# MILAB-IIT-CV/ATDN_vSLAM

Measured on AMD Instinct MI355X. Metric: frame-pairs/sec, KITTI 1241x376 odometry inference at 1/2/4/8 MI355X, higher is better.
Workload: dtype f32 via 3xf16 split MFMA (fp32 accumulate); 1 GPU; KITTI seq-03-shaped 376x1241 uint8 frames (resident in HBM) resized to 376x1232, GMA flow 12 GRU iters + CLVO head -> 6-DoF trajectory (BASELINE configs[1]); streams_per_gpu=2, gru_iters=12, parallelism=pairs sharded x1, one all-gather of 512-d features, replicated LSTM scan

## Files before the change

atdn_vslam_amd/csrc/capi.hip:

```cpp
#include "../../include/atdn_hip.h"

#include <cmath>
#include <cstring>

#include "clvo.h"
#include "gma.h"
#include "vae.h"
#include "clvo_train.h"
#include "frontend.h"
#include "conv_sf.h"
#include "epilogues_sf.h"

namespace atdn {
extern template TileChoice conv_dispatch<MODE_TAP, EpiBias<ACT_NONE>>(const ConvShape&, EpiBias<ACT_NONE>, hipStream_t);
extern template TileChoice conv_dispatch<MODE_TAP, EpiBias<ACT_RELU>>(const ConvShape&, EpiBias<ACT_RELU>, hipStream_t);
extern template TileChoice conv_dispatch<MODE_ROW, EpiBias<ACT_NONE>>(const ConvShape&, EpiBias<ACT_NONE>, hipStream_t);
extern template TileChoice conv_dispatch<MODE_ROW, EpiBias<ACT_RELU>>(const ConvShape&, EpiBias<ACT_RELU>, hipStream_t);
extern template TileChoice conv_dispatch<MODE_TAP, EpiScale>(const ConvShape&, EpiScale, hipStream_t);

extern template TileChoice conv_sf_dispatch<EpiBias<ACT_NONE>>(const ConvShape&, float, EpiBias<ACT_NONE>, hipStream_t);
extern template TileChoice conv_sf_dispatch<SfBias<ACT_NONE>>(const ConvShape&, float, SfBias<ACT_NONE>, hipStream_t);

static thread_local std::string g_last_error;
void set_last_error(const std::string& msg) { g_last_error = msg; }
// ... 518 lines not shown
  ATDN_API_BEGIN
  ATDN_CHECK(src && dst && planes >= 1 && Hin >= 1 && Win >= 1 && Hout >= 1 && Wout >= 1, "bad argument");
  ATDN_CHECK(antialias == 0 || antialias == 1, "antialias must be ATDN_RESIZE_BILINEAR or ATDN_RESIZE_ANTIALIAS");
  launch_resize<unsigned char>(src, planes, Hin, Win, Hout, Wout, antialias, dst, (hipStream_t)stream);
  ATDN_API_END
}
int atdn_pad_frames(const float* src, int planes, int H, int W, int left, int right, int top, int bottom, float* dst,
                    void* stream) {
  ATDN_API_BEGIN
  ATDN_CHECK(src && dst && planes >= 1 && H >= 1 && W >= 1 && left >= 0 && right >= 0 && top >= 0 && bottom >= 0, "bad argument");
  launch_pad_replicate(src, planes, H, W, left, right, top, bottom, dst, (hipStream_t)stream);
  ATDN_API_END
}
int atdn_ingest_create(atdn_ingest** out, int Hin, int Win, int Hout, int Wout, int max_frames, int antialias) {
  ATDN_API_BEGIN
  ATDN_CHECK(out, "null out pointer");
  ATDN_CHECK(antialias == 0 || antialias == 1, "antialias must be ATDN_RESIZE_BILINEAR or ATDN_RESIZE_ANTIALIAS");
  *out = new atdn_ingest(Hin, Win, Hout, Wout, max_frames, antialias);
  ATDN_API_END
}
int atdn_ingest_frames_u8(atdn_ingest* h, const uint8_t* host_frames, int n_frames, float* dst, void* stream) {
  ATDN_API_BEGIN
  ATDN_CHECK(h, "null handle");
  h->in.ingest(host_frames, n_frames, dst, (hipStream_t)stream);
  ATDN_API_END
}
void atdn_ingest_destroy(atdn_ingest* h) { delete h; }

int atdn_conv2d_nhwc_sf_epi(const float* src, int nimg, int H, int W, int Cin, const float* weight_host,
                            const float* bias_host, int Cout, int KH, int KW, int stride, int padH, int padW, int sf_store,
                            float* dst, void* stream) {
  ATDN_API_BEGIN
  ATDN_CHECK(src && weight_host && dst && nimg >= 1 && Cin % 32 == 0, "bad argument (Cin must be a multiple of 32)");
  ATDN_CHECK(!sf_store || Cout % 32 == 0, "the split-f16 store needs Cout % 32 == 0");
  StateDict sd;
  const int64_t ws[4] = {Cout, Cin, KH, KW};
  sd.put("c.weight", weight_host, ws, 4);
  std::vector<float> zb(Cout, 0.f);
  const int64_t bs[1] = {Cout};
  sd.put("c.bias", bias_host ? bias_host : zb.data(), bs, 1);
  WeightArena A;
  PackedConv L = pack_conv_sf(A, sd, {"c"});
  A.upload();
  resolve(A, L);
  hipStream_t st = (hipStream_t)stream;
  float* tmp = nullptr;
  const long rows = (long)nimg * H * W;
  ATDN_HIP(hipMalloc(&tmp, (size_t)rows * Cin * sizeof(float)));
  try {
    launch_to_sf(src, tmp, rows, Cin, st);
    ConvShape s;
    s.src0 = tmp; s.ld0 = Cin; s.sb0 = (long)H * W * Cin; s.C0 = L.C; s.H = H; s.W = W;
    s.KH = KH; s.KW = KW; s.stride = stride; s.padH = padH; s.padW = padW;
    s.w = L.w; s.ldw = L.ldw; s.N = Cout; s.nimg = nimg;
    const int Ho = conv_out(H, KH, stride, padH), Wo = conv_out(W, KW, stride, padW);
    s.wfrag16 = L.wf16;
    if (sf_store) {
      float* osf = nullptr;
      const long orows = (long)nimg * Ho * Wo;
      ATDN_HIP(hipMalloc(&osf, (size_t)orows * Cout * sizeof(float)));
      try {
        conv_sf_dispatch(s, L.wscale, SfBias<ACT_NONE>{L.b, osf, (long)Ho * Wo * Cout, Cout}, st);
        launch_from_sf(osf, dst, orows, Cout, st);
        ATDN_HIP(hipStreamSynchronize(st));
      } catch (...) {
        (void)hipFree(osf);
        throw;
      }
      (void)hipFree(osf);
    } else {
      conv_sf_dispatch(s, L.wscale, EpiBias<ACT_NONE>{L.b, dst, (long)Ho * Wo * Cout, Cout, 1.f}, st);
      ATDN_HIP(hipStreamSynchronize(st));
    }
  } catch (...) {
    (void)hipFree(tmp);
    A.release();
    throw;
  }
  (void)hipFree(tmp);
  A.release();
  ATDN_API_END
}

int atdn_conv2d_nhwc_sf(const float* src, int nimg, int H, int W, int Cin, const float* weight_host,
                        const float* bias_host, int Cout, int KH, int KW, int stride, int padH, int padW, float* dst,
                        void* stream) {
  return atdn_conv2d_nhwc_sf_epi(src, nimg, H, W, Cin, weight_host, bias_host, Cout, KH, KW, stride, padH, padW, 0, dst, stream);
}

// ... 2 lines not shown
```

atdn_vslam_amd/csrc/conv_mfma.h:

```cpp
#pragma once
#include "common.h"

namespace atdn {

typedef float f32x16 __attribute__((ext_vector_type(16)));

enum { MODE_TAP = 0, MODE_ROW = 1 };

struct ConvGeom {
  const float* src0;
  const float* src1;
  long sb0, sb1;
  int ld0, ld1;
  int C0, C1;
  int H, W, Ho, Wo;
  int KH, KW, stride, padH, padW;
  int cpk;
  int nchunks;
  int log2C;
  const float* w;
  long wb;
  int ldw;
  int N;
  int tiles_per_img, nimg, ntile_n;
// ... 182 lines not shown
          for (int e = 0; e < 16; ++e) {
            const int m = mbase + (e & 3) + 8 * (e >> 2) + 4 * h;
            if (m < HoWo) ep.apply(img, m, n, acc[i][j][e], aux[e]);
          }
        } else if constexpr (epi_bias_arg<Epi>::value) {
#pragma unroll
          for (int e = 0; e < 16; ++e) {
            const int m = mbase + (e & 3) + 8 * (e >> 2) + 4 * h;
            if (m < HoWo) ep.store_c(img, m, n, acc[i][j][e], colj[j]);
          }
        } else {
#pragma unroll
          for (int e = 0; e < 16; ++e) {
            const int m = mbase + (e & 3) + 8 * (e >> 2) + 4 * h;
            if (m < HoWo) ep(img, m, n, acc[i][j][e]);
          }
        }
      }
    }
  }
}

struct ConvShape {
  const float* src0 = nullptr; const float* src1 = nullptr;
  long sb0 = 0, sb1 = 0;
  int ld0 = 0, ld1 = 0, C0 = 0, C1 = 0;
  int H = 1, W = 1;
  int KH = 1, KW = 1, stride = 1, padH = 0, padW = 0;
  const float* w = nullptr; long wb = 0; int ldw = 0;
  const float* wfrag16 = nullptr;
  int N = 0;
  int nimg = 1;
  const float* in_mean = nullptr; const float* in_rstd = nullptr;
};

inline int conv_out(int in, int k, int stride, int pad) { return (in + 2 * pad - k) / stride + 1; }

template <int MODE>
inline ConvGeom make_geom(const ConvShape& s, int BM, int BN) {
  ConvGeom g{};
  g.src0 = s.src0; g.src1 = s.src1; g.sb0 = s.sb0; g.sb1 = s.sb1; g.ld0 = s.ld0; g.ld1 = s.ld1;
  g.C0 = s.C0; g.C1 = s.C1; g.H = s.H; g.W = s.W;
  g.KH = s.KH; g.KW = s.KW; g.stride = s.stride; g.padH = s.padH; g.padW = s.padW;
  g.Ho = conv_out(s.H, s.KH, s.stride, s.padH);
  g.Wo = conv_out(s.W, s.KW, s.stride, s.padW);
  if (MODE == MODE_TAP) {
    ATDN_CHECK(s.C0 % 32 == 0 && s.C1 % 32 == 0 && s.C0 > 0, "TAP mode needs channel counts that are multiples of 32");
    ATDN_CHECK(s.ld0 % 4 == 0 && (s.C1 == 0 || (s.src1 && s.ld1 % 4 == 0)), "TAP mode needs 16-byte aligned pixels");
    g.cpk = s.KW * ((s.C0 + s.C1) / 32);
    g.log2C = 0;
  } else {
    ATDN_CHECK(s.C1 == 0 && s.src1 == nullptr, "ROW mode takes one source");
    ATDN_CHECK(s.C0 >= 4 && (s.C0 & (s.C0 - 1)) == 0 && s.ld0 == s.C0, "ROW mode needs dense power-of-two channels");
    g.cpk = cdiv(s.KW * s.C0, 32);
    int l = 0; while ((1 << l) < s.C0) ++l;
    g.log2C = l;
  }
  g.nchunks = s.KH * g.cpk;
  g.w = s.w; g.wb = s.wb; g.ldw = s.ldw; g.N = s.N;
  ATDN_CHECK(s.ldw % 4 == 0 && s.ldw >= g.nchunks * 32, "weight rows must hold the padded K and be 16-byte aligned");
  ATDN_CHECK(((uintptr_t)s.src0 % 16) == 0 && ((uintptr_t)s.w % 16) == 0 && s.sb0 % 4 == 0 && s.wb % 4 == 0,
             "operands must be 16-byte aligned");
  ATDN_CHECK(g.Ho > 0 && g.Wo > 0 && s.N > 0 && s.nimg > 0, "empty convolution");
  g.nimg = s.nimg;
  g.tiles_per_img = cdiv(g.Ho * g.Wo, BM);
  g.ntile_n = cdiv(s.N, BN);
// ... 18 lines not shown
```

atdn_vslam_amd/csrc/conv_sf6.h:

```cpp
#pragma once
#include <cstdlib>
#include <type_traits>
#include "conv_sf.h"

namespace atdn {

struct Conv2Geom {
  const float* src0; const float* src1;
  long sb0, sb1;
  int ld0, ld1, C0, C1;
  int H, W, Ho, Wo;
  int KH, KW, padH, padW;
  int PH, PW;
  int tiles_x, tiles_y;
  int nimg, ntile_n;
  const float* w; int ldw; int N;
  float wscale;
  const float* in_mean; const float* in_rstd;
};

inline bool conv_halo_eligible(const ConvShape& s) {
  if (s.stride != 1 || s.wb != 0) return false;
  return (s.KH == 3 && s.KW == 3) || (s.KH == 1 && s.KW == 5) || (s.KH == 5 && s.KW == 1);
}

template <class E, class = void> struct epi_gen6 : std::integral_constant<int, 0> {};
template <class E> struct epi_gen6<E, std::void_t<decltype(E::kGen6)>> : std::integral_constant<int, E::kGen6> {};
template <class E, class = void> struct EpiAux4 { struct type {}; };
template <class E> struct EpiAux4<E, std::void_t<typename E::Aux4>> { using type = typename E::Aux4; };
template <class E, class = void> struct epi_flowhead : std::false_type {};
template <class E> struct epi_flowhead<E, std::void_t<decltype(E::kFlowHead)>> : std::bool_constant<E::kFlowHead> {};
template <class E, class = void> struct epi_ring3 : std::false_type {};
template <class E> struct epi_ring3<E, std::void_t<decltype(E::kRing3)>> : std::bool_constant<E::kRing3> {};
template <class E, class = void> struct epi_rawacc : std::false_type {};
template <class E> struct epi_rawacc<E, std::void_t<decltype(E::kRawAcc)>> : std::bool_constant<E::kRawAcc> {};
template <class E, class = void> struct epi_vec4 : std::false_type {};
template <class E> struct epi_vec4<E, std::void_t<decltype(E::kVec4)>> : std::bool_constant<E::kVec4> {};

typedef float f32x4v __attribute__((ext_vector_type(4)));
struct SfAcc { f32x4v b[2][2]; };

#ifdef ATDN_CONV_STAMP
#define ATDN_CONV_STAMP_SLOTS 4096
extern __device__ unsigned long long atdn_conv_stamps_dev[4][ATDN_CONV_STAMP_SLOTS][12];
template <class E> struct conv_stamp_kind : std::integral_constant<int, -1> {};
#endif

template <int TH, int TW, int BN, int WM, int WN, int KH, int KW, class Epi, bool FAST = false, bool NORM = false, int ABL = 0>
__device__ __forceinline__ void conv_sf6_body(const Conv2Geom& g, const Epi& ep, const int bidx) {
  static_assert(ABL == 0 || !NORM, "ablation builds exist for the plain patch loader");
  static_assert(TW == 16, "the 16x16x32 loop is built for 16-pixel tile rows");
  constexpr int NIMG = 2;
  constexpr int NW = WM * WN, NT = NW * 64;
  constexpr int TM = TH * TW / 32 / WM, TN = BN / 32 / WN;
  static_assert(TM * WM * 32 == TH * TW && TN * WN * 32 == BN, "wave grid must tile the block");
  static_assert(32 % TW == 0 || TW % 32 == 0, "a 32-pixel MFMA row tile must cover whole tile rows");
  constexpr int NTAP = KH * KW;
  constexpr int RSTEP = NT / 8;
  constexpr int PROWS = (TH + KH - 1) * (TW + KW - 1);
  constexpr int PW = TW + KW - 1;
  constexpr int NP = (PROWS + RSTEP - 1) / RSTEP;
  constexpr int ROWB = 160;
  constexpr int RS = PW * ROWB;
  constexpr bool SWAP = epi_vec4<Epi>::value;
  constexpr int PSZ = (TH + KH - 1) * RS;
  __shared__ __attribute__((aligned(256))) char Pbytes[NIMG * PSZ];

  const int tid = threadIdx.x;
  const int tiles_img = g.tiles_x * g.tiles_y;
  const int nblk = g.nimg * tiles_img * g.ntile_n;
  const int id = xcd_remap(bidx, nblk);
  const int tile_n = id % g.ntile_n;
  const int tmg = id / g.ntile_n;
  const int img = tmg / tiles_img;
  const int tloc = tmg - img * tiles_img;
  const int ty0 = (tloc / g.tiles_x) * TH, tx0 = (tloc % g.tiles_x) * TW;
  const int n0 = tile_n * BN;
  const int lane = tid & 63, wave = tid >> 6;
#ifdef ATDN_CONV_STAMP
  constexpr int kStamp = conv_stamp_kind<Epi>::value;
  unsigned long long st_r0 = 0, st_t0 = 0, st_t1 = 0, st_t2 = 0, st_bar = 0;
  unsigned long long st_e_slab = 0, st_e_wait = 0, st_e_apply = 0;
  if constexpr (kStamp >= 0) { st_r0 = __builtin_amdgcn_s_memrealtime(); st_t0 = __builtin_amdgcn_s_memtime(); }
#endif

  const int jrow = (tid >> 3) & 7;
  const int s = tid & 7, r0 = !NORM ? tid >> 3 : ((tid >> 6) << 3) + 2 * (jrow & 1) + ((jrow >> 1) & 1) + 4 * (jrow >> 2);
  static_assert((TH + KH - 1) * RS / 16 <= 4096, "LDS offset field");
  unsigned pmeta[NP];
#pragma unroll
  for (int k = 0; k < NP; ++k) {
    const int prow = r0 + RSTEP * k;
    unsigned off = 0;
    const int py = prow / PW, px = prow - py * PW;
    if (prow < PROWS) {
      const int iy = ty0 - g.padH + py, ix = tx0 - g.padW + px;
      if ((unsigned)iy < (unsigned)g.H && (unsigned)ix < (unsigned)g.W) off = (unsigned)(iy * g.W + ix) + 1u;
    }
    pmeta[k] = (off << 12) | (unsigned)((py * RS + px * ROWB + 16 * s) >> 4);
    if (prow >= PROWS) pmeta[k] = pmeta[0];
  }
  const float* s0 = g.src0 + (long)img * g.sb0;
  const float* s1 = g.src1 ? g.src1 + (long)img * g.sb1 : nullptr;
  const int nck = (g.C0 + g.C1) >> 5;

  float4 pr[NP];
  auto fetch_patch = [&](int c) {
    const int cc = c << 5;
    const float* sp; int ld, co;
    if (cc < g.C0) { sp = s0; ld = g.ld0; co = cc; } else { sp = s1; ld = g.ld1; co = cc - g.C0; }
#pragma unroll
    for (int k = 0; k < NP; ++k)
      pr[k] = *reinterpret_cast<const float4*>(sp + (long)((pmeta[k] >> 12) ? (pmeta[k] >> 12) - 1 : 0) * ld + co + 4 * s);
  };
  auto store_patch = [&](int buf) {
#pragma unroll
    for (int k = 0; k < NP; ++k)
      *reinterpret_cast<float4*>(Pbytes + buf * PSZ + ((pmeta[k] & 0xFFFu) << 4)) = keep_if((pmeta[k] >> 12) != 0, pr[k]);
  };
  float4 nmu = make_float4(0.f, 0.f, 0.f, 0.f), nrs = make_float4(1.f, 1.f, 1.f, 1.f);
  auto fetch_norm = [&](int c) {
    nmu = *reinterpret_cast<const float4*>(g.in_mean + (long)img * g.C0 + (c << 5) + 4 * s);
    nrs = *reinterpret_cast<const float4*>(g.in_rstd + (long)img * g.C0 + (c << 5) + 4 * s);
  };
  bool norm_sat = false;
  auto store_row_norm = [&](int buf, int k, float4 mu, float4 rs) {
    const float hi = (pmeta[k] >> 12) != 0 ? 65504.f : 0.f;
    float4 v = pr[k];
    v.x = (v.x - mu.x) * rs.x; v.y = (v.y - mu.y) * rs.y; v.z = (v.z - mu.z) * rs.z; v.w = (v.w - mu.w) * rs.w;
    const float m = fmaxf(fmaxf(v.x, v.y), fmaxf(v.z, v.w));
    norm_sat |= !(m <= 65504.f);
    v.x = __builtin_amdgcn_fmed3f(v.x, 0.f, hi); v.y = __builtin_amdgcn_fmed3f(v.y, 0.f, hi);
    v.z = __builtin_amdgcn_fmed3f(v.z, 0.f, hi); v.w = __builtin_amdgcn_fmed3f(v.w, 0.f, hi);
    const unsigned h0 = sf_cvt_pk_(v.x, v.y), h1 = sf_cvt_pk_(v.z, v.w);
    const unsigned l0 = sf_residual_pk_(h0, v.x, v.y), l1 = sf_residual_pk_(h1, v.z, v.w);
    char* px = Pbytes + buf * PSZ + (((pmeta[k] & 0xFFFu) - (unsigned)s) << 4);
    *reinterpret_cast<uint2*>(px + 8 * s) = make_uint2(h0, h1);
    *reinterpret_cast<uint2*>(px + 64 + 8 * s) = make_uint2(l0, l1);
  };

  const int wm = wave / WN, wn = wave % WN;
  SfAcc acc[TM][TN];
#pragma unroll
  for (int i = 0; i < TM; ++i)
#pragma unroll
    for (int j = 0; j < TN; ++j) {
#pragma unroll
      for (int e = 0; e < 16; ++e) acc[i][j].b[e >> 3][(e >> 2) & 1][e & 3] = 0.f;
    }
  {
    const int n16 = lane & 15, g16 = lane >> 4;
    int a_off[TM];
#pragma unroll
    for (int i = 0; i < TM; ++i) a_off[i] = ((wm * TM + i) * 2) * RS + n16 * ROWB + 16 * g16;
    const char* Pb = Pbytes;
    const int nblk16 = (g.N + 15) >> 4;
    const float* wrow[TN][2];
#pragma unroll
    for (int j = 0; j < TN; ++j)
#pragma unroll
      for (int cb = 0; cb < 2; ++cb)
        wrow[j][cb] = g.w + (long)min(((n0 >> 4) + (wn * TN + j) * 2 + cb), nblk16 - 1) * (NTAP * nck) * 512 + lane * 4;
    constexpr int RT = (NTAP % 3 == 0 || epi_ring3<Epi>::value) ? 3 : 2;
    constexpr int CU = (NTAP % RT == 0) ? 1 : RT;
    constexpr int NS = CU * NTAP;
    static_assert(NS % RT == 0, "ring size must divide the K steps of an unrolled iteration");
    struct WFrag { f16x8 hi[TN][2], lo[TN][2]; };
    WFrag wr[RT];
    auto load_w = [&](WFrag& f, int c0, int st, int cb) __attribute__((always_inline)) {
      const int cc = min(c0 + st / NTAP, nck - 1);
      const int q = (st % NTAP) * nck + cc;
#pragma unroll
      for (int j = 0; j < TN; ++j) {
        f.hi[j][cb] = *reinterpret_cast<const f16x8*>(wrow[j][cb] + (long)q * 512);
        if constexpr (!FAST) f.lo[j][cb] = *reinterpret_cast<const f16x8*>(wrow[j][cb] + (long)q * 512 + 256);
      }
    };
    fetch_patch(0);
    if constexpr (NORM) fetch_norm(0);
#pragma unroll
    for (int st = 0; st < RT - 1; ++st) { load_w(wr[st], 0, st, 0); load_w(wr[st], 0, st, 1); }
    if constexpr ((ABL & 1) != 0) { load_w(wr[RT - 1], 0, RT - 1, 0); load_w(wr[RT - 1], 0, RT - 1, 1); }
    if constexpr (NORM) {
#pragma unroll
      for (int k = 0; k < NP; ++k) store_row_norm(0, k, nmu, nrs);
    } else {
      store_patch(0);
    }
    __syncthreads();
#ifdef ATDN_CONV_STAMP
    if constexpr (kStamp >= 0) st_t1 = __builtin_amdgcn_s_memtime();
#endif
    f16x8 ah[2][TM], al[2][TM];
    auto read_a = [&](int half, int tap) __attribute__((always_inline)) {
      const char* arow = Pb + (tap / KW + half) * RS + (tap % KW) * ROWB;
#pragma unroll
      for (int i = 0; i < TM; ++i) {
        ah[half][i] = *reinterpret_cast<const f16x8*>(arow + a_off[i]);
        if constexpr (!FAST) al[half][i] = *reinterpret_cast<const f16x8*>(arow + a_off[i] + 64);
      }
    };
    auto mfma_half = [&](int half, const WFrag& w) __attribute__((always_inline)) {
#pragma unroll
      for (int i = 0; i < TM; ++i)
#pragma unroll
        for (int j = 0; j < TN; ++j)
#pragma unroll
          for (int cb = 0; cb < 2; ++cb) {
            f32x4v c = acc[i][j].b[half][cb];
            if constexpr (SWAP) {
              if constexpr (!FAST) {
                c = __builtin_amdgcn_mfma_f32_16x16x32_f16(w.hi[j][cb], al[half][i], c, 0, 0, 0);
                c = __builtin_amdgcn_mfma_f32_16x16x32_f16(w.lo[j][cb], ah[half][i], c, 0, 0, 0);
              }
              c = __builtin_amdgcn_mfma_f32_16x16x32_f16(w.hi[j][cb], ah[half][i], c, 0, 0, 0);
            } else {
              if constexpr (!FAST) {
                c = __builtin_amdgcn_mfma_f32_16x16x32_f16(al[half][i], w.hi[j][cb], c, 0, 0, 0);
                c = __builtin_amdgcn_mfma_f32_16x16x32_f16(ah[half][i], w.lo[j][cb], c, 0, 0, 0);
              }
              c = __builtin_amdgcn_mfma_f32_16x16x32_f16(ah[half][i], w.hi[j][cb], c, 0, 0, 0);
            }
            acc[i][j].b[half][cb] = c;
          }
    };
    constexpr int NMF = (FAST ? 1 : 3) * TM * TN * 2;
    constexpr int NH = 2 * NTAP;
    static_assert(!NORM || NH - 1 - NP >= 1, "normalise-on-load spreads its NP patch rows over the half-steps of a chunk");
    read_a(0, 0);
    if constexpr (KH != 3 || !Epi::kStats) __builtin_amdgcn_s_setprio(2);
    for (int c0 = 0; c0 < nck; c0 += CU) {
#pragma unroll
// ... 53 lines not shown
    if constexpr (kStamp >= 0) {
      asm volatile("s_waitcnt vmcnt(0) lgkmcnt(0)" ::: "memory");
      const unsigned long long t3 = __builtin_amdgcn_s_memtime(), r1 = __builtin_amdgcn_s_memrealtime();
      const unsigned hw = __builtin_amdgcn_s_getreg((31 << 11) | 4), xcc = __builtin_amdgcn_s_getreg((31 << 11) | 20);
      if (wave == 0 && lane == 0 && bidx < ATDN_CONV_STAMP_SLOTS) {
        unsigned long long* o = atdn_conv_stamps_dev[kStamp * 2 + (KH == 5 ? 1 : 0)][bidx];
        o[0] = st_r0; o[1] = r1; o[2] = st_t1 - st_t0; o[3] = st_t2 - st_t1; o[4] = st_bar; o[5] = t3 - st_t2;
        o[6] = ((unsigned long long)xcc << 32) | hw; o[7] = t3 - st_t0;
        o[8] = st_e_slab; o[9] = st_e_wait; o[10] = st_e_apply; o[11] = 0;
      }
    }
  };
#endif
  if constexpr (KH != 3 || !Epi::kStats) __builtin_amdgcn_s_setprio(0);
  if constexpr (NORM) sf_report(norm_sat);
  if constexpr ((ABL & 8) != 0) {
    float tot = 0.f;
#pragma unroll
    for (int i = 0; i < TM; ++i)
#pragma unroll
      for (int j = 0; j < TN; ++j)
#pragma unroll
        for (int e = 0; e < 16; ++e) tot += acc[i][j].b[e >> 3][(e >> 2) & 1][e & 3];
    if (tot == 1.2345e-30f) ep(img, 0, 0, tot);
    return;
  }
  if constexpr (SWAP) {
    static_assert(NW * 32 * LDS_LD * 4 <= NIMG * PSZ, "transpose slabs must fit in the patch images");
    __syncthreads();
    float* tb = reinterpret_cast<float*>(Pbytes) + wave * (32 * LDS_LD);
    const int trow = lane >> 3, tcol = (lane & 7) * 4;
    auto tile_pixel = [&](int i, int q) {
      const int p = (wm * TM + i) * 32 + 8 * q + trow;
      const int oy = ty0 + p / TW, ox = tx0 + p % TW;
      if constexpr ((ABL & 16) != 0) return p;
      return (oy < g.Ho && ox < g.Wo) ? oy * g.Wo + ox : -1;
    };
    constexpr bool RAW = epi_rawacc<Epi>::value && !epi_flowhead<Epi>::value;
    auto slab_write = [&](const SfAcc& a) __attribute__((always_inline)) {
      const float sc = RAW ? 1.0f : g.wscale;
#pragma unroll
      for (int hh = 0; hh < 2; ++hh)
#pragma unroll
        for (int cb = 0; cb < 2; ++cb)
          *reinterpret_cast<float4*>(tb + (16 * hh + (lane & 15)) * LDS_LD + 16 * cb + 4 * (lane >> 4)) =
              RAW ? make_float4(a.b[hh][cb][0], a.b[hh][cb][1], a.b[hh][cb][2], a.b[hh][cb][3])
                  : make_float4(a.b[hh][cb][0] * sc, a.b[hh][cb][1] * sc, a.b[hh][cb][2] * sc, a.b[hh][cb][3] * sc);
    };
    if constexpr (epi_flowhead<Epi>::value) {
      static_assert(!epi_flowhead<Epi>::value || (WM == 1 && TN == 1 && TW == 16), "one block holds all output channels of its pixels");
      constexpr int RP = 20;
      static_assert(32 * RP <= 32 * LDS_LD, "the exchange rows live inside the wave's slab");
      {
        const int n16 = lane & 15, g16 = lane >> 4;
        const int c8 = n0 + wn * 32 + 8 * g16;
        const float4 bq0 = *reinterpret_cast<const float4*>(ep.bias + c8), bq1 = *reinterpret_cast<const float4*>(ep.bias + c8 + 4);
        const float b8[8] = {bq0.x, bq0.y, bq0.z, bq0.w, bq1.x, bq1.y, bq1.z, bq1.w};
        f16x8 w2h[2], w2l[2];
#pragma unroll
        for (int rbk = 0; rbk < 2; ++rbk) {
          const int u = 16 * rbk + n16;
          const float* wr = ep.w2 + (long)min(u, 17) * g.N + c8;
          const float4 wa = *reinterpret_cast<const float4*>(wr), wb = *reinterpret_cast<const float4*>(wr + 4);
          const float w8[8] = {wa.x, wa.y, wa.z, wa.w, wb.x, wb.y, wb.z, wb.w};
#pragma unroll
          for (int e = 0; e < 8; ++e) {
            const float w = u < 18 ? w8[e] * ep.w2mul : 0.f;
            w2h[rbk][e] = (_Float16)w;
            w2l[rbk][e] = (_Float16)(w - (float)w2h[rbk][e]);
// ... 138 lines not shown
                if (nb + e < g.N) ep(img, mq[q], nb + e, e4[e]);
            }
          }
        }
      }
    }
    sf_report(clamped);
#ifdef ATDN_CONV_STAMP
    stamp_out();
#endif
    return;
  }
  constexpr int NSET = 2, NPX = 8;
  auto col_of = [&](int cs) { return 16 * cs + (lane & 15); };
  auto pix_of = [&](int e) { return 16 * (e >> 2) + 4 * (lane >> 4) + (e & 3); };
  auto val_of = [&](const SfAcc& a, int cs, int e) __attribute__((always_inline)) { return a.b[e >> 2][cs][e & 3]; };
  typename EpiCol<Epi>::type colj[TN][NSET];
  float biasj[TN][NSET];
#pragma unroll
  for (int j = 0; j < TN; ++j)
#pragma unroll
    for (int cs = 0; cs < NSET; ++cs) {
      const int n = min(n0 + (wn * TN + j) * 32 + col_of(cs), g.N - 1);
      biasj[j][cs] = 0.f;
      if constexpr (Epi::kStats) biasj[j][cs] = ep.bias[n];
      if constexpr (epi_bias_arg<Epi>::value) colj[j][cs] = ep.col(n);
    }
#pragma unroll
  for (int i = 0; i < TM; ++i) {
    const int pbase = (wm * TM + i) * 32;
    int mm[NPX];
#pragma unroll
    for (int e = 0; e < NPX; ++e) {
      const int p = pbase + pix_of(e);
      const int oy = ty0 + p / TW, ox = tx0 + p % TW;
      mm[e] = (oy < g.Ho && ox < g.Wo) ? oy * g.Wo + ox : -1;
    }
    int cnt = 0;
    unsigned mo[NPX];
    if constexpr (Epi::kStats) {
#pragma unroll
      for (int e = 0; e < NPX; ++e) {
        cnt += mm[e] >= 0 ? 1 : 0;
        mo[e] = (unsigned)max(mm[e], 0) * (unsigned)ep.ld;
      }
      cnt += __shfl_xor(cnt, 16);
      cnt += __shfl_xor(cnt, 32);
      cnt = __builtin_amdgcn_readfirstlane(cnt);
    }
    const bool full = cnt == 32;
    const float inv_cnt = 1.0f / (float)(cnt > 0 ? cnt : 1);
#pragma unroll
    for (int j = 0; j < TN; ++j)
#pragma unroll
      for (int cs = 0; cs < NSET; ++cs) {
        const int n = n0 + (wn * TN + j) * 32 + col_of(cs);
        const bool nok = n < g.N;
        if constexpr (Epi::kStats) {
          const float bias = nok ? biasj[j][cs] : 0.f;
          float v[NPX];
#pragma unroll
          for (int e = 0; e < NPX; ++e) v[e] = __builtin_fmaf(val_of(acc[i][j], cs, e), g.wscale, bias);
          float sum, m2;
          if (full) {
            sum = ((v[0] + v[1]) + (v[2] + v[3])) + ((v[4] + v[5]) + (v[6] + v[7]));
          } else {
            sum = 0.f;
#pragma unroll
            for (int e = 0; e < NPX; ++e) sum += mm[e] >= 0 ? v[e] : 0.f;
// ... 25 lines not shown
          if (nok) {
            char* ob = reinterpret_cast<char*>(ep.dst + (long)img * ep.ob);
#pragma unroll
            for (int e = 0; e < NPX; ++e)
              if (full || mm[e] >= 0) *reinterpret_cast<float*>(ob + 4u * (mo[e] + (unsigned)n)) = v[e];
          }
          continue;
        }
        if (nok) {
          if constexpr (Epi::kPrefetch) {
            typename Epi::Aux aux[NPX];
#pragma unroll
            for (int e = 0; e < NPX; ++e) aux[e] = ep.load(img, max(mm[e], 0), n);
#pragma unroll
            for (int e = 0; e < NPX; ++e)
              if (mm[e] >= 0) ep.apply(img, mm[e], n, val_of(acc[i][j], cs, e) * g.wscale, aux[e]);
          } else if constexpr (epi_bias_arg<Epi>::value) {
#pragma unroll
            for (int e = 0; e < NPX; ++e)
              if (mm[e] >= 0) ep.store_c(img, mm[e], n, val_of(acc[i][j], cs, e) * g.wscale, colj[j][cs]);
          } else {
#pragma unroll
            for (int e = 0; e < NPX; ++e)
              if (mm[e] >= 0) ep(img, mm[e], n, val_of(acc[i][j], cs, e) * g.wscale);
          }
        }
      }
  }
}

template <int TH, int TW, int BN, int WM, int WN, int KH, int KW, class Epi, bool FAST = false, bool NORM = false, int ABL = 0>
__global__ __launch_bounds__(WM * WN * 64, 1) void conv_sf6_kernel(const Conv2Geom g, const Epi ep) {
  conv_sf6_body<TH, TW, BN, WM, WN, KH, KW, Epi, FAST, NORM, ABL>(g, ep, (int)blockIdx.x);
}

__device__ __forceinline__ Conv2Geom conv2_geom_pick(const Conv2Geom& a, const Conv2Geom& b, bool s) {
  Conv2Geom g;
  g.src0 = s ? b.src0 : a.src0; g.src1 = s ? b.src1 : a.src1; g.sb0 = s ? b.sb0 : a.sb0; g.sb1 = s ? b.sb1 : a.sb1;
  g.ld0 = s ? b.ld0 : a.ld0; g.ld1 = s ? b.ld1 : a.ld1; g.C0 = s ? b.C0 : a.C0; g.C1 = s ? b.C1 : a.C1;
  g.H = s ? b.H : a.H; g.W = s ? b.W : a.W; g.Ho = s ? b.Ho : a.Ho; g.Wo = s ? b.Wo : a.Wo;
  g.KH = s ? b.KH : a.KH; g.KW = s ? b.KW : a.KW; g.padH = s ? b.padH : a.padH; g.padW = s ? b.padW : a.padW;
  g.PH = s ? b.PH : a.PH; g.PW = s ? b.PW : a.PW; g.tiles_x = s ? b.tiles_x : a.tiles_x; g.tiles_y = s ? b.tiles_y : a.tiles_y;
  g.nimg = s ? b.nimg : a.nimg; g.ntile_n = s ? b.ntile_n : a.ntile_n;
  g.w = s ? b.w : a.w; g.ldw = s ? b.ldw : a.ldw; g.N = s ? b.N : a.N; g.wscale = s ? b.wscale : a.wscale;
  g.in_mean = nullptr; g.in_rstd = nullptr;
  return g;
}
template <int TH, int TW, int BN, int WM, int WN, int KH, int KW, class Epi, bool FAST = false>
__global__ __launch_bounds__(WM * WN * 64, 1) void conv_sf6_pair_kernel(const Conv2Geom g0, const Conv2Geom g1, const Epi ep0,
                                                                        const Epi ep1, const int nblk0, const int start1) {
  const int b = (int)blockIdx.x;
  if (b >= nblk0 && b < start1) return;
  const bool second = b >= start1;
  const Conv2Geom g = conv2_geom_pick(g0, g1, second);
  const Epi ep = Epi::pick(ep0, ep1, second);
  conv_sf6_body<TH, TW, BN, WM, WN, KH, KW, Epi, FAST, false, 0>(g, ep, second ? b - start1 : b);
}

template <int TH, int BN, int WM, int WN, int KH, int KW, class Epi, bool FAST = false, bool NORM = false, int ABL = 0>
inline Conv2Geom conv_sf6_geom(const ConvShape& s, float wscale) {
  constexpr int TW = 16;
  ATDN_CHECK(s.KH == KH && s.KW == KW && s.stride == 1, "kernel shape does not match the instantiation");
  Conv2Geom g{};
  g.src0 = s.src0; g.src1 = s.src1; g.sb0 = s.sb0; g.sb1 = s.sb1; g.ld0 = s.ld0; g.ld1 = s.ld1;
  g.C0 = s.C0; g.C1 = s.C1; g.H = s.H; g.W = s.W;
  g.KH = s.KH; g.KW = s.KW; g.padH = s.padH; g.padW = s.padW;
  g.Ho = conv_out(s.H, s.KH, 1, s.padH); g.Wo = conv_out(s.W, s.KW, 1, s.padW);
  g.PH = TH + s.KH - 1; g.PW = TW + s.KW - 1;
  ATDN_CHECK(s.C0 % 32 == 0 && s.C1 % 32 == 0 && s.C0 > 0 && s.ld0 % 4 == 0, "TAP-mode channel constraints");
  ATDN_CHECK(s.ldw % 4 == 0 && s.ldw >= s.KH * s.KW * (s.C0 + s.C1), "weight rows too short");
  ATDN_CHECK(!epi_vec4<Epi>::value || !Epi::kPrefetch || s.N % 4 == 0, "channel-vector epilogue with operand loads needs N % 4 == 0");
  ATDN_CHECK((long)s.H * s.W < (1L << 20) - 1, "image too large for the packed patch descriptor");
  ATDN_CHECK((long)g.Ho * g.Wo * 1024L * 4L <= (1L << 32) && s.ld0 <= 1024 && s.ld1 <= 1024 && s.N <= 1024,
             "per-image slice of 4 GB or more: the 32-bit epilogue offsets would wrap");
  g.tiles_x = cdiv(g.Wo, TW); g.tiles_y = cdiv(g.Ho, TH);
  g.nimg = s.nimg; g.ntile_n = cdiv(s.N, BN);
  g.w = s.wfrag16; g.ldw = s.ldw; g.N = s.N; g.wscale = wscale;
  g.in_mean = s.in_mean; g.in_rstd = s.in_rstd;
  ATDN_CHECK(NORM == (s.in_mean != nullptr) && (!NORM || (s.in_rstd && s.C1 == 0 && s.ld0 == s.C0)),
             "normalise-on-load: one dense fp32 source with its mean / rstd");
  ATDN_CHECK(g.w != nullptr, "missing weight copy for this kernel");
  return g;
}

template <int TH, int BN, int WM, int WN, int KH, int KW, class Epi, bool FAST = false, bool NORM = false, int ABL = 0>
inline void launch_conv_sf6(const ConvShape& s, float wscale, Epi ep, hipStream_t st) {
  constexpr int TW = 16;
  const Conv2Geom g = conv_sf6_geom<TH, BN, WM, WN, KH, KW, Epi, FAST, NORM, ABL>(s, wscale);
  set_groups(ep, g.tiles_x * g.tiles_y * (TH * TW / 32));
  const int nblk = g.nimg * g.tiles_x * g.tiles_y * g.ntile_n;
  hipLaunchKernelGGL((conv_sf6_kernel<TH, TW, BN, WM, WN, KH, KW, Epi, FAST, NORM, ABL>), dim3(nblk), dim3(WM * WN * 64), 0, st, g, ep);
  ATDN_HIP(hipGetLastError());
}

template <int TH, int BN, int WM, int WN, int KH, int KW, class Epi, bool FAST>
inline void launch_conv_sf6_pair(const ConvShape& s0, float wscale0, Epi ep0, const ConvShape& s1, float wscale1, Epi ep1,
                                 hipStream_t st) {
  constexpr int TW = 16;
  static_assert(!Epi::kStats, "the pair launch serves plain-store epilogues");
  const Conv2Geom g0 = conv_sf6_geom<TH, BN, WM, WN, KH, KW, Epi, FAST, false, 0>(s0, wscale0);
  const Conv2Geom g1 = conv_sf6_geom<TH, BN, WM, WN, KH, KW, Epi, FAST, false, 0>(s1, wscale1);
  const int nblk0 = g0.nimg * g0.tiles_x * g0.tiles_y * g0.ntile_n;
  const int start1 = (nblk0 + 7) / 8 * 8;
  const int nblk1 = g1.nimg * g1.tiles_x * g1.tiles_y * g1.ntile_n;
  hipLaunchKernelGGL((conv_sf6_pair_kernel<TH, TW, BN, WM, WN, KH, KW, Epi, FAST>), dim3(start1 + nblk1), dim3(WM * WN * 64), 0, st,
                     g0, g1, ep0, ep1, nblk0, start1);
  ATDN_HIP(hipGetLastError());
}


inline int conv_sf6_block_width_3x3(const ConvShape& s) {
  const int Ho = conv_out(s.H, s.KH, 1, s.padH), Wo = conv_out(s.W, s.KW, 1, s.padW);
  const long tiles = (long)s.nimg * cdiv(Wo, 16) * cdiv(Ho, 8);
  int bn = 64;
  if (s.N <= 32) bn = 32;
  else if (s.N == 96) bn = 96;
  else {
    int best = cdiv(s.N, 64) * 64;
    for (int c : {128, 256})
      if (cdiv(s.N, c) * c <= best) { best = cdiv(s.N, c) * c; bn = c; }
  }
  while (bn > 64 && bn != 96 && tiles * cdiv(s.N, bn) < 300) bn /= 2;
  return bn;
}

template <int TH, int BN, int WM, int WN, int KH, int KW, class Epi, bool FAST, bool NORM>
inline void launch_conv_sf6_m(const ConvShape& s, float wscale, const Epi& ep, hipStream_t st) {
  launch_conv_sf6<TH, BN, WM, WN, KH, KW, Epi, FAST, NORM>(s, wscale, ep, st);
}

template <int KH, int KW, class Epi, bool FAST>
inline bool conv_sf6_try_shape(const ConvShape& s, float wscale, const Epi& ep, hipStream_t st, int* bn_out, int* th_out) {
  const int Ho = conv_out(s.H, s.KH, 1, s.padH), Wo = conv_out(s.W, s.KW, 1, s.padW);
  const long tiles = (long)s.nimg * cdiv(Wo, 16) * cdiv(Ho, 8);
  int bn = 64;
  if (s.N <= 32 && KH == 3) bn = 32;
  else if (s.N == 96 && KH == 3) bn = 96;
  else {
    int best = cdiv(s.N, 64) * 64;
    for (int c : {128, 256})
      if (cdiv(s.N, c) * c <= best) { best = cdiv(s.N, c) * c; bn = c; }
  }
  while (bn > 64 && bn != 96 && tiles * cdiv(s.N, bn) < 300) bn /= 2;
  if constexpr (KH != 3) bn = std::min(bn, 128);
  *th_out = 8;
  if (s.in_mean) {
    if constexpr (Epi::kStats && KH == 3 && !FAST) {
      const bool tall = (bn == 64 || bn == 96) && cdiv(Ho, 12) * 12 * 100 <= cdiv(Ho, 8) * 8 * 103;
      *bn_out = bn; *th_out = tall ? 12 : 8;
      if (bn == 64 && tall) launch_conv_sf6_m<12, 64, 2, 2, KH, KW, Epi, false, true>(s, wscale, ep, st);
      else if (bn == 64) launch_conv_sf6_m<8, 64, 2, 2, KH, KW, Epi, false, true>(s, wscale, ep, st);
      else if (bn == 96 && tall) launch_conv_sf6_m<12, 96, 2, 3, KH, KW, Epi, false, true>(s, wscale, ep, st);
      else if (bn == 96) launch_conv_sf6_m<8, 96, 2, 3, KH, KW, Epi, false, true>(s, wscale, ep, st);
      else if (bn == 128) launch_conv_sf6_m<8, 128, 1, 4, KH, KW, Epi, false, true>(s, wscale, ep, st);
      else return false;
      return true;
    } else {
      return false;
    }
  }
  if constexpr (!Epi::kStats && !epi_flowhead<Epi>::value) {
    static const bool force_small = getenv("ATDN_CONV_SMALL_TILES") && getenv("ATDN_CONV_SMALL_TILES")[0] == '1';
    if ((bn == 64 && tiles * cdiv(s.N, 64) < 300) || (force_small && KH != 3)) {
      *bn_out = 64; *th_out = 4;
      launch_conv_sf6_m<4, 64, 2, 2, KH, KW, Epi, FAST, false>(s, wscale, ep, st);
      return true;
    }
  }
  if constexpr (KH != 3 && !Epi::kStats && !epi_flowhead<Epi>::value) {
    static const bool half128 = getenv("ATDN_CONV_SMALL_TILES") && getenv("ATDN_CONV_SMALL_TILES")[0] == '2';
    if (half128 && bn == 128) {
      *bn_out = 128; *th_out = 4;
      launch_conv_sf6_m<4, 128, 1, 4, KH, KW, Epi, FAST, false>(s, wscale, ep, st);
      return true;
    }
  }
  if constexpr (KH == 3) {
    if (bn == 32) { *bn_out = 32; launch_conv_sf6_m<8, 32, 4, 1, KH, KW, Epi, FAST, false>(s, wscale, ep, st); return true; }
    const long tiles12 = (long)s.nimg * cdiv(Wo, 16) * cdiv(Ho, 12);
    const bool tall = (bn == 64 || bn == 96) && cdiv(Ho, 12) * 12 * 100 <= cdiv(Ho, 8) * 8 * 103 &&
                      (Epi::kStats || tiles12 * cdiv(s.N, bn) >= 512);
    if (tall) {
      *bn_out = bn; *th_out = 12;
      if (bn == 64) launch_conv_sf6_m<12, 64, 2, 2, KH, KW, Epi, FAST, false>(s, wscale, ep, st);
      else launch_conv_sf6_m<12, 96, 2, 3, KH, KW, Epi, FAST, false>(s, wscale, ep, st);
      return true;
    }
  }
  *bn_out = bn;
  switch (bn) {
    case 64:  launch_conv_sf6_m<8, 64, 2, 2, KH, KW, Epi, FAST, false>(s, wscale, ep, st); return true;
    case 128: launch_conv_sf6_m<8, 128, 1, 4, KH, KW, Epi, FAST, false>(s, wscale, ep, st); return true;
    case 256: launch_conv_sf6_m<8, 256, 1, 8, KH, KW, Epi, FAST, false>(s, wscale, ep, st); return true;
    default: break;
  }
  if constexpr (KH == 3) {
    if (bn == 96) { launch_conv_sf6_m<8, 96, 2, 3, KH, KW, Epi, FAST, false>(s, wscale, ep, st); return true; }
  }
  return false;
}

template <class Epi>
inline bool conv_sf6_try_pair(const ConvShape& s0, float wscale0, const Epi& ep0, const ConvShape& s1, float wscale1, const Epi& ep1,
                              hipStream_t st, bool fast) {
  if constexpr ((epi_gen6<Epi>::value & 1) == 0 || Epi::kStats || epi_flowhead<Epi>::value) {
    return false;
  } else {
    auto picks_tall64 = [&](const ConvShape& s) {
      if (!conv_halo_eligible(s) || s.KH != 3 || s.KW != 3 || !s.wfrag16 || s.in_mean) return false;
      if (epi_vec4<Epi>::value && (s.N % 4) != 0) return false;
      if (s.C0 % 32 != 0 || s.C1 % 32 != 0 || s.C0 <= 0 || s.ld0 % 4 != 0) return false;
      if (conv_sf6_block_width_3x3(s) != 64) return false;
      const int Ho = conv_out(s.H, 3, 1, s.padH), Wo = conv_out(s.W, 3, 1, s.padW);
      const long tiles12 = (long)s.nimg * cdiv(Wo, 16) * cdiv(Ho, 12);
      return cdiv(Ho, 12) * 12 * 100 <= cdiv(Ho, 8) * 8 * 103 && tiles12 * cdiv(s.N, 64) >= 512;
    };
    if (!picks_tall64(s0) || !picks_tall64(s1)) return false;
    if (fast) launch_conv_sf6_pair<12, 64, 2, 2, 3, 3, Epi, true>(s0, wscale0, ep0, s1, wscale1, ep1, st);
    else launch_conv_sf6_pair<12, 64, 2, 2, 3, 3, Epi, false>(s0, wscale0, ep0, s1, wscale1, ep1, st);
    return true;
  }
}
// ... 26 lines not shown
```

atdn_vslam_amd/csrc/conv_sf_inst_a.hip:

```cpp
#include "conv_sf_dispatch_impl.h"
namespace atdn {
ATDN_INSTANTIATE_CONV_SF(SfBias<ACT_NONE>)
ATDN_INSTANTIATE_CONV_SF(SfBias<ACT_RELU>)
ATDN_INSTANTIATE_CONV_SF(EpiBias<ACT_NONE>)
ATDN_INSTANTIATE_CONV_SF_PAIR(SfBias<ACT_RELU>)
}
```

atdn_vslam_amd/csrc/epilogues_sf.h:

```cpp
#pragma once
#include "epilogues.h"
#include "sf.h"

namespace atdn {

template <int ACT>
struct SfBias {
  static constexpr bool kStats = false;
  static constexpr bool kPrefetch = false;
  const float* bias;
  float* dst; long ob; int ld;
  static __device__ __forceinline__ SfBias pick(const SfBias& a, const SfBias& b, bool second) {
    return SfBias{second ? b.bias : a.bias, second ? b.dst : a.dst, second ? b.ob : a.ob, second ? b.ld : a.ld};
  }
  __device__ __forceinline__ void operator()(int img, int m, int n, float a) const { store_c(img, m, n, a, col(n)); }
  struct Col { float b; };
  __device__ __forceinline__ Col col(int n) const { return {bias ? bias[n] : 0.f}; }
  __device__ __forceinline__ void store_c(int img, int m, int n, float a, Col c) const {
    float v = a + c.b;
    if (ACT == ACT_RELU) v = fmaxf(v, 0.f);
    sf_store(dst, (long)img * ob + (long)m * ld, n, v);
  }
  static constexpr bool kVec4 = true;
  static constexpr int kGen6 = 1;
  __device__ __forceinline__ float4 bias4(int n) const {
    return bias ? *reinterpret_cast<const float4*>(bias + n) : make_float4(0.f, 0.f, 0.f, 0.f);
  }
  __device__ __forceinline__ void store4(int img, int m, int n, float4 a, float4 b, bool& clamped) const {
    a.x += b.x; a.y += b.y; a.z += b.z; a.w += b.w;
    if (ACT == ACT_RELU) { a.x = fmaxf(a.x, 0.f); a.y = fmaxf(a.y, 0.f); a.z = fmaxf(a.z, 0.f); a.w = fmaxf(a.w, 0.f); }
    sf_store4_flag(dst, (long)img * ob + (long)m * ld, n, a, clamped);
  }
};

struct SfBiasReluAddRelu {
  static constexpr bool kStats = false;
  static constexpr bool kPrefetch = true;
  const float* bias;
  const float* res; long rb; int ldr;
  float* dst; long ob; int ld;
  struct Aux { float r; };
  __device__ __forceinline__ Aux load(int img, int m, int n) const { return {sf_load(res, (long)img * rb + (long)m * ldr, n)}; }
  __device__ __forceinline__ void apply(int img, int m, int n, float a, Aux x) const {
    const float y = fmaxf(a + bias[n], 0.f);
    sf_store(dst, (long)img * ob + (long)m * ld, n, fmaxf(x.r + y, 0.f));
  }
  static constexpr bool kVec4 = true;
  static constexpr int kGen6 = 1;
  struct Aux4 { float4 r; };
  __device__ __forceinline__ Aux4 load4(int img, int m, int n) const { return {sf_load4(res, (long)img * rb + (long)m * ldr, n)}; }
  __device__ __forceinline__ float4 bias4(int n) const { return *reinterpret_cast<const float4*>(bias + n); }
  __device__ __forceinline__ void apply4(int img, int m, int n, float4 a, Aux4 x, float4 b, bool& clamped) const {
    float4 o;
    o.x = fmaxf(x.r.x + fmaxf(a.x + b.x, 0.f), 0.f);
    o.y = fmaxf(x.r.y + fmaxf(a.y + b.y, 0.f), 0.f);
    o.z = fmaxf(x.r.z + fmaxf(a.z + b.z, 0.f), 0.f);
    o.w = fmaxf(x.r.w + fmaxf(a.w + b.w, 0.f), 0.f);
// ... 159 lines not shown
```

Before: 418.3 frame-pairs/s.

## Add run-tile kernel for separable 1x5/5x1 convolutions along image rows

```diff
diff --git a/atdn_vslam_amd/csrc/capi.hip b/atdn_vslam_amd/csrc/capi.hip
--- a/atdn_vslam_amd/csrc/capi.hip
+++ b/atdn_vslam_amd/csrc/capi.hip
@@ -574,6 +574,9 @@
                             float* dst, void* stream) {
   ATDN_API_BEGIN
   ATDN_CHECK(src && weight_host && dst && nimg >= 1 && Cin % 32 == 0, "bad argument (Cin must be a multiple of 32)");
+  ATDN_CHECK(sf_store >= 0 && sf_store <= 7 && (sf_store & 6) != 6, "sf_store: bit 0 names the epilogue, bit 1 or bit 2 the tile form");
+  const int tile_form = (sf_store & 2) ? 1 : (sf_store & 4) ? 2 : 0;
+  sf_store &= 1;
   ATDN_CHECK(!sf_store || Cout % 32 == 0, "the split-f16 store needs Cout % 32 == 0");
   StateDict sd;
   const int64_t ws[4] = {Cout, Cin, KH, KW};
@@ -597,6 +600,7 @@
     s.w = L.w; s.ldw = L.ldw; s.N = Cout; s.nimg = nimg;
     const int Ho = conv_out(H, KH, stride, padH), Wo = conv_out(W, KW, stride, padW);
     s.wfrag16 = L.wf16;
+    s.tile_form = tile_form;
     if (sf_store) {
       float* osf = nullptr;
       const long orows = (long)nimg * Ho * Wo;
diff --git a/atdn_vslam_amd/csrc/conv_mfma.h b/atdn_vslam_amd/csrc/conv_mfma.h
--- a/atdn_vslam_amd/csrc/conv_mfma.h
+++ b/atdn_vslam_amd/csrc/conv_mfma.h
@@ -238,6 +238,7 @@
   int N = 0;
   int nimg = 1;
   const float* in_mean = nullptr; const float* in_rstd = nullptr;
+  int tile_form = 0;
 };
 
 inline int conv_out(int in, int k, int stride, int pad) { return (in + 2 * pad - k) / stride + 1; }
diff --git a/atdn_vslam_amd/csrc/conv_sf6.h b/atdn_vslam_amd/csrc/conv_sf6.h
--- a/atdn_vslam_amd/csrc/conv_sf6.h
+++ b/atdn_vslam_amd/csrc/conv_sf6.h
@@ -46,9 +46,13 @@
 template <class E> struct conv_stamp_kind : std::integral_constant<int, -1> {};
 #endif
 
-template <int TH, int TW, int BN, int WM, int WN, int KH, int KW, class Epi, bool FAST = false, bool NORM = false, int ABL = 0>
+template <int TH, int TW, int BN, int WM, int WN, int KH, int KW, class Epi, bool FAST = false, bool NORM = false, int ABL = 0,
+          bool RUN = false>
 __device__ __forceinline__ void conv_sf6_body(const Conv2Geom& g, const Epi& ep, const int bidx) {
   static_assert(ABL == 0 || !NORM, "ablation builds exist for the plain patch loader");
+  static_assert(!RUN || (((KH == 1 && KW == 5) || (KH == 5 && KW == 1)) && TH == 8 && BN == 128 && WM == 1 && WN == 4 && !NORM &&
+                         ABL == 0 && !Epi::kStats && !epi_flowhead<Epi>::value),
+                "run tiles: separable passes on the 8 x 16 x 128 block, plain loader, epilogues without statistics");
   static_assert(TW == 16, "the 16x16x32 loop is built for 16-pixel tile rows");
   constexpr int NIMG = 2;
   constexpr int NW = WM * WN, NT = NW * 64;
@@ -57,13 +61,14 @@
   static_assert(32 % TW == 0 || TW % 32 == 0, "a 32-pixel MFMA row tile must cover whole tile rows");
   constexpr int NTAP = KH * KW;
   constexpr int RSTEP = NT / 8;
-  constexpr int PROWS = (TH + KH - 1) * (TW + KW - 1);
+  constexpr int RSLOTS = 160;
+  constexpr int PROWS = RUN ? RSLOTS : (TH + KH - 1) * (TW + KW - 1);
   constexpr int PW = TW + KW - 1;
   constexpr int NP = (PROWS + RSTEP - 1) / RSTEP;
   constexpr int ROWB = 160;
   constexpr int RS = PW * ROWB;
   constexpr bool SWAP = epi_vec4<Epi>::value;
-  constexpr int PSZ = (TH + KH - 1) * RS;
+  constexpr int PSZ = RUN ? RSLOTS * ROWB : (TH + KH - 1) * RS;
   __shared__ __attribute__((aligned(256))) char Pbytes[NIMG * PSZ];
 
   const int tid = threadIdx.x;
@@ -77,6 +82,21 @@
   const int ty0 = (tloc / g.tiles_x) * TH, tx0 = (tloc % g.tiles_x) * TW;
   const int n0 = tile_n * BN;
   const int lane = tid & 63, wave = tid >> 6;
+  const int rL = KH == 1 ? g.W : g.H, rHW = g.H * g.W;
+  const int rm0 = tloc * (TH * TW);
+  const int rrun0 = RUN ? rm0 / rL : 0, rpos0 = rm0 - rrun0 * rL;
+  const int rb1 = rL - rpos0, rb2 = rb1 + rL, rb3 = rb2 + rL;
+  auto out_pixel = [&](int p) {
+    if constexpr (RUN) {
+      const int k = (p >= rb1 ? 1 : 0) + (p >= rb2 ? 1 : 0) + (p >= rb3 ? 1 : 0);
+      const int m = rm0 + p;
+      if (m >= rHW) return -1;
+      return KH == 1 ? m : (rpos0 + p - k * rL) * g.W + rrun0 + k;
+    } else {
+      const int oy = ty0 + p / TW, ox = tx0 + p % TW;
+      return (oy < g.Ho && ox < g.Wo) ? oy * g.Wo + ox : -1;
+    }
+  };
 #ifdef ATDN_CONV_STAMP
   constexpr int kStamp = conv_stamp_kind<Epi>::value;
   unsigned long long st_r0 = 0, st_t0 = 0, st_t1 = 0, st_t2 = 0, st_bar = 0;
@@ -86,12 +106,22 @@
 
   const int jrow = (tid >> 3) & 7;
   const int s = tid & 7, r0 = !NORM ? tid >> 3 : ((tid >> 6) << 3) + 2 * (jrow & 1) + ((jrow >> 1) & 1) + 4 * (jrow >> 2);
-  static_assert((TH + KH - 1) * RS / 16 <= 4096, "LDS offset field");
+  static_assert(PSZ / 16 <= 4096, "LDS offset field");
   unsigned pmeta[NP];
 #pragma unroll
   for (int k = 0; k < NP; ++k) {
     const int prow = r0 + RSTEP * k;
     unsigned off = 0;
+    if constexpr (RUN) {
+      static_assert(PROWS == NP * RSTEP, "every loader step writes slots of the image");
+      const int kk = (prow >= 2 + rb1 ? 1 : 0) + (prow >= 10 + rb2 ? 1 : 0) + (prow >= 18 + rb3 ? 1 : 0);
+      const bool gap = kk > 0 && prow < 2 + rb1 + (kk - 1) * rL + 8 * kk;
+      const int p = prow - 2 - 8 * kk;
+      const int pos = rpos0 + p - kk * rL;
+      if (!gap && p < 130 && (unsigned)pos < (unsigned)rL && rm0 + p < rHW) off = (unsigned)(KH == 1 ? rm0 + p : pos * g.W + rrun0 + kk) + 1u;
+      pmeta[k] = (off << 12) | (unsigned)((prow * ROWB + 16 * s) >> 4);
+      continue;
+    }
     const int py = prow / PW, px = prow - py * PW;
     if (prow < PROWS) {
       const int iy = ty0 - g.padH + py, ix = tx0 - g.padW + px;
@@ -150,9 +180,20 @@
     }
   {
     const int n16 = lane & 15, g16 = lane >> 4;
-    int a_off[TM];
-#pragma unroll
-    for (int i = 0; i < TM; ++i) a_off[i] = ((wm * TM + i) * 2) * RS + n16 * ROWB + 16 * g16;
+    int a_off[RUN ? 2 * TM : TM];
+#pragma unroll
+    for (int i = 0; i < TM; ++i) {
+      if constexpr (RUN) {
+#pragma unroll
+        for (int hh = 0; hh < 2; ++hh) {
+          const int p = ((wm * TM + i) * 2 + hh) * 16 + n16;
+          const int k = (p >= rb1 ? 1 : 0) + (p >= rb2 ? 1 : 0) + (p >= rb3 ? 1 : 0);
+          a_off[hh * TM + i] = (p + 8 * k) * ROWB + 16 * g16;
+        }
+      } else {
+        a_off[i] = ((wm * TM + i) * 2) * RS + n16 * ROWB + 16 * g16;
+      }
+    }
     const char* Pb = Pbytes;
     const int nblk16 = (g.N + 15) >> 4;
     const float* wrow[TN][2];
@@ -193,11 +234,12 @@
 #endif
     f16x8 ah[2][TM], al[2][TM];
     auto read_a = [&](int half, int tap) __attribute__((always_inline)) {
-      const char* arow = Pb + (tap / KW + half) * RS + (tap % KW) * ROWB;
+      const char* arow = RUN ? Pb + tap * ROWB : Pb + (tap / KW + half) * RS + (tap % KW) * ROWB;
 #pragma unroll
       for (int i = 0; i < TM; ++i) {
-        ah[half][i] = *reinterpret_cast<const f16x8*>(arow + a_off[i]);
-        if constexpr (!FAST) al[half][i] = *reinterpret_cast<const f16x8*>(arow + a_off[i] + 64);
+        const int ao = a_off[RUN ? half * TM + i : i];
+        ah[half][i] = *reinterpret_cast<const f16x8*>(arow + ao);
+        if constexpr (!FAST) al[half][i] = *reinterpret_cast<const f16x8*>(arow + ao + 64);
       }
     };
     auto mfma_half = [&](int half, const WFrag& w) __attribute__((always_inline)) {
@@ -317,9 +359,8 @@
     const int trow = lane >> 3, tcol = (lane & 7) * 4;
     auto tile_pixel = [&](int i, int q) {
       const int p = (wm * TM + i) * 32 + 8 * q + trow;
-      const int oy = ty0 + p / TW, ox = tx0 + p % TW;
       if constexpr ((ABL & 16) != 0) return p;
-      return (oy < g.Ho && ox < g.Wo) ? oy * g.Wo + ox : -1;
+      return out_pixel(p);
     };
     constexpr bool RAW = epi_rawacc<Epi>::value && !epi_flowhead<Epi>::value;
     auto slab_write = [&](const SfAcc& a) __attribute__((always_inline)) {
@@ -524,9 +565,7 @@
     int mm[NPX];
 #pragma unroll
     for (int e = 0; e < NPX; ++e) {
-      const int p = pbase + pix_of(e);
-      const int oy = ty0 + p / TW, ox = tx0 + p % TW;
-      mm[e] = (oy < g.Ho && ox < g.Wo) ? oy * g.Wo + ox : -1;
+      mm[e] = out_pixel(pbase + pix_of(e));
     }
     int cnt = 0;
     unsigned mo[NPX];
@@ -618,6 +657,11 @@
 template <int TH, int TW, int BN, int WM, int WN, int KH, int KW, class Epi, bool FAST = false, bool NORM = false, int ABL = 0>
 __global__ __launch_bounds__(WM * WN * 64, 1) void conv_sf6_kernel(const Conv2Geom g, const Epi ep) {
   conv_sf6_body<TH, TW, BN, WM, WN, KH, KW, Epi, FAST, NORM, ABL>(g, ep, (int)blockIdx.x);
+}
+
+template <int KH, int KW, class Epi, bool FAST = false>
+__global__ __launch_bounds__(256, 1) void conv_sf6_run_kernel(const Conv2Geom g, const Epi ep) {
+  conv_sf6_body<8, 16, 128, 1, 4, KH, KW, Epi, FAST, false, 0, true>(g, ep, (int)blockIdx.x);
 }
 
 __device__ __forceinline__ Conv2Geom conv2_geom_pick(const Conv2Geom& a, const Conv2Geom& b, bool s) {
@@ -679,6 +723,24 @@
   ATDN_HIP(hipGetLastError());
 }
 
+template <int KH, int KW>
+inline bool conv_sf6_run_eligible(const ConvShape& s) {
+  if (KH * KW != 5 || s.KH != KH || s.KW != KW || s.stride != 1 || s.in_mean) return false;
+  if (s.padH != KH / 2 || s.padW != KW / 2) return false;
+  const int L = KH == 1 ? s.W : s.H;
+  return (L + 126) / L <= 3;
+}
+
+template <int KH, int KW, class Epi, bool FAST>
+inline void launch_conv_sf6_run(const ConvShape& s, float wscale, Epi ep, hipStream_t st) {
+  Conv2Geom g = conv_sf6_geom<8, 128, 1, 4, KH, KW, Epi, FAST, false, 0>(s, wscale);
+  ATDN_CHECK((conv_sf6_run_eligible<KH, KW>(s)) && g.Ho == g.H && g.Wo == g.W, "shape not served by the run-tile kernel");
+  g.tiles_x = cdiv(g.H * g.W, 128); g.tiles_y = 1;
+  const int nblk = g.nimg * g.tiles_x * g.ntile_n;
+  hipLaunchKernelGGL((conv_sf6_run_kernel<KH, KW, Epi, FAST>), dim3(nblk), dim3(256), 0, st, g, ep);
+  ATDN_HIP(hipGetLastError());
+}
+
 template <int TH, int BN, int WM, int WN, int KH, int KW, class Epi, bool FAST>
 inline void launch_conv_sf6_pair(const ConvShape& s0, float wscale0, Epi ep0, const ConvShape& s1, float wscale1, Epi ep1,
                                  hipStream_t st) {
@@ -745,6 +807,22 @@
       return false;
     }
   }
+  if constexpr (KH != 3 && !Epi::kStats && !epi_flowhead<Epi>::value) {
+    if (s.tile_form == 1) {
+      *bn_out = 128;
+      launch_conv_sf6_m<8, 128, 1, 4, KH, KW, Epi, FAST, false>(s, wscale, ep, st);
+      return true;
+    }
+    if (s.tile_form == 2 && conv_sf6_run_eligible<KH, KW>(s)) {
+#ifndef ATDN_NO_RUN_TILES
+      *bn_out = 128;
+      launch_conv_sf6_run<KH, KW, Epi, FAST>(s, wscale, ep, st);
+      return true;
+#else
+      ATDN_CHECK(false, "run tiles requested from a library built with ATDN_NO_RUN_TILES");
+#endif
+    }
+  }
   if constexpr (!Epi::kStats && !epi_flowhead<Epi>::value) {
     static const bool force_small = getenv("ATDN_CONV_SMALL_TILES") && getenv("ATDN_CONV_SMALL_TILES")[0] == '1';
     if ((bn == 64 && tiles * cdiv(s.N, 64) < 300) || (force_small && KH != 3)) {
@@ -774,6 +852,11 @@
     }
   }
   *bn_out = bn;
+#ifndef ATDN_NO_RUN_TILES
+  if constexpr (KH != 3 && !Epi::kStats && !epi_flowhead<Epi>::value) {
+    if (bn == 128 && conv_sf6_run_eligible<KH, KW>(s)) { launch_conv_sf6_run<KH, KW, Epi, FAST>(s, wscale, ep, st); return true; }
+  }
+#endif
   switch (bn) {
     case 64:  launch_conv_sf6_m<8, 64, 2, 2, KH, KW, Epi, FAST, false>(s, wscale, ep, st); return true;
     case 128: launch_conv_sf6_m<8, 128, 1, 4, KH, KW, Epi, FAST, false>(s, wscale, ep, st); return true;
diff --git a/atdn_vslam_amd/csrc/conv_sf_inst_a.hip b/atdn_vslam_amd/csrc/conv_sf_inst_a.hip
--- a/atdn_vslam_amd/csrc/conv_sf_inst_a.hip
+++ b/atdn_vslam_amd/csrc/conv_sf_inst_a.hip
@@ -1,6 +1,5 @@
 #include "conv_sf_dispatch_impl.h"
 namespace atdn {
-ATDN_INSTANTIATE_CONV_SF(SfBias<ACT_NONE>)
 ATDN_INSTANTIATE_CONV_SF(SfBias<ACT_RELU>)
 ATDN_INSTANTIATE_CONV_SF(EpiBias<ACT_NONE>)
 ATDN_INSTANTIATE_CONV_SF_PAIR(SfBias<ACT_RELU>)
diff --git a/atdn_vslam_amd/csrc/conv_sf_inst_f.hip b/atdn_vslam_amd/csrc/conv_sf_inst_f.hip
--- /dev/null
+++ b/atdn_vslam_amd/csrc/conv_sf_inst_f.hip
@@ -0,0 +1,4 @@
+#include "conv_sf_dispatch_impl.h"
+namespace atdn {
+ATDN_INSTANTIATE_CONV_SF(SfBias<ACT_NONE>)
+}
diff --git a/atdn_vslam_amd/csrc/epilogues_sf.h b/atdn_vslam_amd/csrc/epilogues_sf.h
--- a/atdn_vslam_amd/csrc/epilogues_sf.h
+++ b/atdn_vslam_amd/csrc/epilogues_sf.h
@@ -22,7 +22,7 @@
     sf_store(dst, (long)img * ob + (long)m * ld, n, v);
   }
   static constexpr bool kVec4 = true;
-  static constexpr int kGen6 = 1;
+  static constexpr int kGen6 = ACT == ACT_NONE ? 3 : 1;
   __device__ __forceinline__ float4 bias4(int n) const {
     return bias ? *reinterpret_cast<const float4*>(bias + n) : make_float4(0.f, 0.f, 0.f, 0.f);
   }
```

New measurement: 424.1 frame-pairs/s, median of 6. +1.4%, better.
